# TheJacksonLaboratory/cnn_autoencoder

Measured on AMD Instinct MI355X. Metric: tiles/sec, compress+decompress round trip of 1024x1024x3 histology tiles, higher is better.
Workload: dtype f32 (f16x3 split MFMA: 3 f16 MFMAs per product, fp32 accumulate)

## Files before the change

cnn_autoencoder_amd/csrc/cae_api.hip:

```cpp
#include "cae_hip.h"
#include "cae_internal.hpp"
#include "cae_kernels.hpp"
#include "cae_kernels_f16.hpp"
#include "cae_launch.hpp"
#include "cae_pack.hpp"

#include <algorithm>
#include <cmath>
#include <cstdio>
#include <cstdlib>
#include <cstring>
#include <string>

namespace cae {

thread_local std::string g_last_error;
thread_local int64_t g_last_ticket = 0;
thread_local int g_force_fp32 = 0;

int fail(int code, const char *fmt, ...) {
    char buf[512];
    va_list ap;
    va_start(ap, fmt);
    vsnprintf(buf, sizeof buf, fmt, ap);
// ... 74 lines not shown
            if (l.set && l.f16_bad) return false;
    return true;
}

Model::~Model() {
    if (order_event) (void)hipEventDestroy((hipEvent_t)order_event);
    if (flags) (void)hipHostFree(flags);
}

struct ProfScope {
    Model *m;
    int track;
    hipStream_t st;
    std::vector<std::pair<void *, void *>> ev;
    hipEvent_t cur = nullptr;
    ProfScope(Model *m_, int track_, hipStream_t st_) : m(m_), track(track_), st(st_) {}
    void begin() {
        if (!m->profiling) return;
        hipEvent_t a;
        if (hipEventCreate(&a) != hipSuccess) return;
        (void)hipEventRecord(a, st);
        cur = a;
    }
    void end() {
        if (!m->profiling || !cur) return;
        hipEvent_t b;
        if (hipEventCreate(&b) != hipSuccess) return;
        (void)hipEventRecord(b, st);
        ev.emplace_back((void *)cur, (void *)b);
        cur = nullptr;
    }
    ~ProfScope() {
        if (m->profiling && !ev.empty()) m->prof[track].push_back(std::move(ev));
    }
};

static unsigned ew_grid(size_t total) {
    size_t b = (total + 255) / 256;
    return (unsigned)std::min<size_t>(std::max<size_t>(b, 1), 256 * 8 * 4);
}

static int layer_of(Model *m, int track, int index, Layer *&l) {
    if (track != CAE_ANALYSIS && track != CAE_SYNTHESIS) return fail(CAE_ERR_ARG, "bad track %d", track);
    if (index < 0 || index >= m->L) return fail(CAE_ERR_ARG, "layer index %d out of range", index);
    l = &(track == CAE_ANALYSIS ? m->enc : m->dec)[index];
    return CAE_OK;
}

static int upload_channels(DevBuf &d, const float *v, int c, int ct, float fill) {
    if (!v) {
        d.reset();
        return CAE_OK;
    }
    return d.upload(pad_channels(v, c, ct, fill));
}

static LayerArgs layer_args(const Model *m, const float *in, int in_planes, void *out, int n, int h, int w, int oh, int ow,
                            int ct, int cout, int outfmt, int act, int *flag) {
    LayerArgs a{};
    a.in = in;
    a.out = out;
    a.zero = m->zero.get<float>();
    a.medians = m->zero.get<float>();
    a.flag = flag;
    a.N = n;
    a.H = h;
    a.W = w;
    a.OH = oh;
    a.OW = ow;
    a.in_planes = in_planes;
    a.out_planes = ct * 4;
    a.cout = cout;
    a.outfmt = outfmt;
    a.act = act;
    return a;
}

}

using namespace cae;

template <int R>
static void launch_likelihood(Model *m, const float *y, int n, int hw, float *yhat, float *lik, double *part,
                              hipStream_t st) {
    hipLaunchKernelGGL(likelihood_kernel<R>, dim3(m->c_bn, n), dim3(256), 0, st, y, m->medians_dev.get<float>(),
                       m->density_dev.get<float>(), m->density_per_channel, m->density_k, m->density_bound,
                       m->likelihood_plain, m->c_bn, hw, yhat, lik, part);
}

static int set_stage(Model *m, int track, Layer &l, int stage, const float *w, const float *bias, const float *beta,
                     const float *gamma, int act, int add_residual, int post_act) {
    const int ctin = round_ct(l.cin);
    if (ctin < 0) return fail(CAE_ERR_UNSUPPORTED, "more than 192 channels not supported");
    if ((int)l.stages.size() <= stage) l.stages.resize(stage + 1);
    Layer::Stage &sg = l.stages[stage];
    const bool tr = track == CAE_SYNTHESIS;
    CAE_TRY(sg.wp.upload(pack_weights(w, tr, l.cin, l.cin, m->ks, ctin, tr)));
    CAE_TRY(upload_channels(sg.bias, bias, l.cin, ctin, 0.0f));
    sg.gdn = beta != nullptr;
    if (sg.gdn) {
        CAE_TRY(upload_channels(sg.beta, beta, l.cin, ctin, 1.0f));
        CAE_TRY(sg.gp.upload(pack_gamma(gamma, l.cin, ctin)));
    }
    sg.act = act;
    sg.add_res = add_residual != 0;
    sg.post_act = post_act;
    if (m->precision == 1) {
// ... 970 lines not shown
```

cnn_autoencoder_amd/csrc/cae_kernels.hpp:

```cpp
#pragma once
#include <hip/hip_runtime.h>
#include <stdint.h>
#include <type_traits>
#include <utility>

namespace cae {

typedef float f32x16 __attribute__((ext_vector_type(16)));
typedef float f32x4 __attribute__((ext_vector_type(4)));

enum OutFmt { OUT_C8 = 0, OUT_NCHW = 1, OUT_U8HWC = 2, OUT_SYM = 3, OUT_PMAP = 4 };

struct LayerArgs {
    const float *in;
    void *out;
    const float *wp;
    const float *bias;
    const float *gp;
    const float *beta;
    const float *zero;
    int N, H, W, OH, OW;
    int in_planes;
    int cci;
    int out_planes;
    int cout;
    int tiles_x, tiles_y;
    int outfmt;
    int act;
    const float *res;
    int res_planes;
    int post_act;
    const float *medians;
    const void *pm;
    int *flag;
};

__device__ __forceinline__ uint8_t clip_u8(float q) {
    return (uint8_t)__builtin_fmaxf(__builtin_fminf(q, 255.0f), 0.0f);
}
__device__ __forceinline__ int round_sym(float d) {
    return (int)rintf(__builtin_fminf(__builtin_fmaxf(d, -1073741824.0f), 1073741824.0f));
}

template <int N, class F, int... I>
__device__ __forceinline__ void static_for_impl(F &&f, std::integer_sequence<int, I...>) {
    (f(std::integral_constant<int, I>{}), ...);
}
template <int N, class F>
__device__ __forceinline__ void static_for(F &&f) {
    static_for_impl<N>(static_cast<F &&>(f), std::make_integer_sequence<int, N>{});
}

__device__ __forceinline__ int reflect_idx(int i, int n) {
    i = i < 0 ? -i : i;
    i = i >= n ? 2 * n - 2 - i : i;
    i = i < 0 ? 0 : i;
    return i >= n ? n - 1 : i;
}

__device__ __forceinline__ void glds16(const void *gsrc, void *lds_wave_base) {
    __builtin_amdgcn_global_load_lds((const __attribute__((address_space(1))) void *)gsrc,
                                     (__attribute__((address_space(3))) void *)lds_wave_base, 16, 0, 0);
}

__device__ __forceinline__ void wait_vm0() { asm volatile("s_waitcnt vmcnt(0)" ::: "memory"); }

__device__ __forceinline__ constexpr int acc_row(int r) { return (r & 3) + 8 * (r >> 2); }

template <int CT>
__device__ __forceinline__ void init_acc(f32x16 (&acc)[CT], const float *vec, int h, float fill) {
#pragma unroll
    for (int ct = 0; ct < CT; ++ct)
#pragma unroll
        for (int r = 0; r < 16; ++r) acc[ct][r] = vec ? vec[32 * ct + acc_row(r) + 4 * h] : fill;
}

template <int CT, int NW, bool INVERSE, int STAGE_BYTES, class Tail>
__device__ __forceinline__ void gdn_stages(f32x16 (&y)[CT], const LayerArgs &p, char *smem, int &sc,
                                           int wave, int lane, Tail tail) {
    constexpr int G_BYTES = CT * 4096;
    const int h = lane >> 5;
    f32x16 nrm[CT];
    init_acc<CT>(nrm, p.beta, h, 1.0f);
#pragma unroll
    for (int jt = 0; jt < CT; ++jt) {
        wait_vm0();
        __syncthreads();
        char *cur = smem + (sc & 1) * STAGE_BYTES;
        char *nxt = smem + ((sc + 1) & 1) * STAGE_BYTES;
        const char *gb = cur + lane * 16;
        f32x4 g_cur[CT];
#pragma unroll
        for (int co = 0; co < CT; ++co) g_cur[co] = *(const f32x4 *)(gb + (co * 4) * 1024);
        if (jt + 1 < CT) {
            const char *src = (const char *)p.gp + (size_t)(jt + 1) * G_BYTES;
#pragma unroll
            for (int i = 0; i < (CT * 4 + NW - 1) / NW; ++i) {
                const int j = wave + i * NW;
                if (j < CT * 4) glds16(src + j * 1024 + lane * 16, nxt + j * 1024);
            }
        } else {
            tail(nxt);
        }
#pragma unroll
        for (int q = 0; q < 4; ++q) {
            f32x4 g_nxt[CT];
            if (q + 1 < 4) {
#pragma unroll
                for (int co = 0; co < CT; ++co) g_nxt[co] = *(const f32x4 *)(gb + (co * 4 + q + 1) * 1024);
            }
            __builtin_amdgcn_sched_barrier(0);
#pragma unroll
            for (int jj = 0; jj < 4; ++jj) {
                const float v = y[jt][4 * q + jj];
                const float sq = v * v;
#pragma unroll
                for (int co = 0; co < CT; ++co)
                    nrm[co] = __builtin_amdgcn_mfma_f32_32x32x2f32(g_cur[co][jj], sq, nrm[co], 0, 0, 0);
            }
            if (q + 1 < 4) {
#pragma unroll
                for (int co = 0; co < CT; ++co) g_cur[co] = g_nxt[co];
            }
        }
        ++sc;
    }
#pragma unroll
// ... 1087 lines not shown
```

cnn_autoencoder_amd/csrc/cae_kernels_f16.hpp:

```cpp
#pragma once
#include "cae_kernels.hpp"

namespace cae {

constexpr int F16_ISSUERS = 2;
#define ISSUER(w, NW, NI) ((w) < (NI) ? (w) : -1)

typedef _Float16 f16x8 __attribute__((ext_vector_type(8)));
typedef _Float16 f16x4 __attribute__((ext_vector_type(4)));


__device__ __forceinline__ void split_f16(float v, _Float16 &hi, _Float16 &lo) {
    hi = (_Float16)v;
    lo = (_Float16)(v - (float)hi);
}

typedef unsigned u32x2v __attribute__((ext_vector_type(2)));
__device__ __forceinline__ u32x2v split2_f16(float a, float b) {
    typedef float f32x2 __attribute__((ext_vector_type(2)));
    typedef _Float16 f16x2 __attribute__((ext_vector_type(2)));
    const f32x2 ab = {a, b};
    const unsigned hi = __builtin_bit_cast(unsigned, __builtin_convertvector(ab, f16x2));
    float l0, l1;
    asm("v_fma_mix_f32 %0, %1, -1.0, %2 op_sel_hi:[1,0,0]" : "=v"(l0) : "v"(hi), "v"(a));
// ... 292 lines not shown
    int sc = 0;

    issue_stage(0, std::integral_constant<int, 0>{}, smem);
    for (int q = 0; q < p.cci; ++q) {
        static_for<KS>([&](auto ky_tag) {
            constexpr int ky = decltype(ky_tag)::value;
            wait_vm0();
            __syncthreads();
            char *cur = smem + (sc & 1) * STAGE_BYTES;
            char *nxt = smem + ((sc + 1) & 1) * STAGE_BYTES;
            if constexpr (ky + 1 < KS) {
                issue_stage(q, std::integral_constant<int, ky + 1>{}, nxt);
            } else {
                if (q + 1 < p.cci) {
                    issue_stage(q + 1, std::integral_constant<int, 0>{}, nxt);
                } else if (GDN) {
                    issue_gamma0<CT, NW>(p, nxt, wave, lane);
                }
            }
            const char *wb = cur + lane * 16;
            const char *hb = cur + b_off;
#pragma unroll
            for (int kx = 0; kx < KS; ++kx) {
                const int kxr = kx;
                f16x8 bh[PT], bl[PT];
#pragma unroll
                for (int pt = 0; pt < PT; ++pt) {
                    bh[pt] = *(const f16x8 *)(hb + pt * B_PT + kxr * 16);
                    bl[pt] = *(const f16x8 *)(hb + pt * B_PT + kxr * 16 + B_HL);
                }
#pragma unroll
                for (int ct = 0; ct < CT; ++ct) {
                    const f16x8 ah = *(const f16x8 *)(wb + ((kxr * CT + ct) * 2 + 0) * 1024);
                    const f16x8 al = *(const f16x8 *)(wb + ((kxr * CT + ct) * 2 + 1) * 1024);
#pragma unroll
                    for (int pt = 0; pt < PT; ++pt) acc[pt][ct] = mfma3(ah, al, bh[pt], bl[pt], acc[pt][ct]);
                }
            }
            ++sc;
        });
    }

    if constexpr (GDN) {
        gdn_stages_f16<CT, PT, NW, ZP, STAGE_BYTES>(acc, p, smem, sc, wave, lane, [](char *) {});
    }
#pragma unroll
    for (int pt = 0; pt < PT; ++pt) {
        const int oy = oy0 + 2 * PT * wave + 2 * pt + (m >> 4), ox = ox0 + (m & 15);
        store_tiles_f16<CT, SP, (GDN ? 0 : 1) | (RES ? 2 : 0)>(acc[pt], p, n, oy, ox, h, oy < p.OH && ox < p.OW);
    }
}

template <int CT, bool INVERSE>
__device__ __forceinline__ void gdn_resident_f16(f32x16 (&y)[CT], const char *gbuf, const float *beta_lds, int lane) {
    const int h = lane >> 5;
    f32x16 nrm[CT];
    float mx = 0.0f;
#pragma unroll
    for (int ct = 0; ct < CT; ++ct)
#pragma unroll
        for (int r = 0; r < 16; r += 2)
            mx = absmax3(mx, y[ct][r], y[ct][r + 1]);
    float isc;
    const float sc = pixel_scale(mx, &isc), sc2 = sc * sc;
#pragma unroll
    for (int ct = 0; ct < CT; ++ct)
#pragma unroll
        for (int r = 0; r < 16; ++r) nrm[ct][r] = beta_lds[32 * ct + acc_row(r) + 4 * h] * sc2;
#pragma unroll
    for (int jt = 0; jt < CT; ++jt) {
        const char *gb = gbuf + jt * (CT * 4096) + lane * 16;
#pragma unroll
        for (int s = 0; s < 2; ++s) {
            __builtin_amdgcn_sched_barrier(0);
            u32x4v hw, lw;
#pragma unroll
            for (int e = 0; e < 4; ++e) {
                const float v0 = y[jt][8 * s + 2 * e] * sc, v1 = y[jt][8 * s + 2 * e + 1] * sc;
                { const u32x2v t_ = split2_f16(v0 * v0, v1 * v1); hw[e] = t_[0]; lw[e] = t_[1]; }
                if constexpr (!INVERSE) {
                    y[jt][8 * s + 2 * e] = v0;
                    y[jt][8 * s + 2 * e + 1] = v1;
                }
            }
            const f16x8 sh = __builtin_bit_cast(f16x8, hw), sl = __builtin_bit_cast(f16x8, lw);
#pragma unroll
            for (int co = 0; co < CT; ++co) {
                if (co & 1) __builtin_amdgcn_sched_barrier(0);
                const f16x8 gh = *(const f16x8 *)(gb + ((co * 2 + s) * 2 + 0) * 1024);
                const f16x8 gl = *(const f16x8 *)(gb + ((co * 2 + s) * 2 + 1) * 1024);
                nrm[co] = mfma3(gh, gl, sh, sl, nrm[co]);
            }
        }
    }
#pragma unroll
    for (int ct = 0; ct < CT; ++ct)
#pragma unroll
        for (int r = 0; r < 16; ++r) {
            const float nv = nrm[ct][r];
            if constexpr (INVERSE)
                y[ct][r] *= __builtin_amdgcn_sqrtf(nv) * isc;
            else
                y[ct][r] *= __builtin_amdgcn_rsqf(nv);
        }
}

template <int CT, bool INVERSE>
__device__ __forceinline__ void gdn_resident_pipe_f16(f32x16 (&y)[CT], const char *gbuf, const float *beta_lds, int lane) {
    const int h = lane >> 5;
    f32x16 nrm[CT];
    float mx = 0.0f;
#pragma unroll
    for (int ct = 0; ct < CT; ++ct)
#pragma unroll
        for (int r = 0; r < 16; r += 2)
            mx = absmax3(mx, y[ct][r], y[ct][r + 1]);
    float isc;
    const float sc = pixel_scale(mx, &isc), sc2 = sc * sc;
#pragma unroll
    for (int ct = 0; ct < CT; ++ct)
#pragma unroll
// ... 55 lines not shown
                y[ct][r] *= __builtin_amdgcn_rsqf(nv);
        }
}

template <int CT, bool INVERSE, bool SP>
__global__ void __launch_bounds__(256, 1) gdn_f16_kernel(const LayerArgs p) {
    constexpr int NW = 4;
    extern __shared__ __attribute__((aligned(16))) char smem[];
    char *gbuf = smem;
    float *beta_lds = (float *)(smem + CT * CT * 4096);
    const int lane = threadIdx.x & 63;
    const int wave = __builtin_amdgcn_readfirstlane(threadIdx.x >> 6);
    const int h = lane >> 5, m = lane & 31;
    for (int j = wave; j < CT * CT * 4; j += NW) glds16((const char *)p.gp + (size_t)j * 1024 + lane * 16, gbuf + j * 1024);
    for (int i = threadIdx.x; i < CT * 32; i += NW * 64) beta_lds[i] = p.beta[i];
    wait_vm0();
    __syncthreads();

    const int groups = (int)(c8s_row_bytes<SP>(p.OW) / 1024);
    const long total = (long)p.N * p.OH * groups;
    const size_t row_bytes = c8s_row_bytes<SP>(p.OW);
    char *base = (char *)p.out;
    for (long t = (long)blockIdx.x * NW + wave; t < total; t += (long)gridDim.x * NW) {
        const int g = (int)(t % groups);
        const long rest = t / groups;
        const int oy = (int)(rest % p.OH), n = (int)(rest / p.OH);
        const int ox = SP ? (g >> 1) * 64 + 2 * m + (g & 1) : g * 32 + m;
        const bool valid = ox < p.OW;
        f32x16 y[CT];
#pragma unroll
        for (int ct = 0; ct < CT; ++ct)
#pragma unroll
            for (int pl = 0; pl < 4; ++pl) {
                const size_t row = ((size_t)n * p.out_planes + 4 * ct + pl) * p.OH + oy;
                const char *src = base + row * row_bytes + (size_t)g * 1024 + m * 16 + 8 * h;
                const f16x4 vh = *(const f16x4 *)src, vl = *(const f16x4 *)(src + 512);
#pragma unroll
                for (int k = 0; k < 4; ++k) y[ct][4 * pl + k] = valid ? (float)vh[k] + (float)vl[k] : 0.0f;
            }
        float mx = 0.0f;
#pragma unroll
        for (int ct = 0; ct < CT; ++ct)
#pragma unroll
            for (int r = 0; r < 16; r += 2)
                mx = absmax3(mx, y[ct][r], y[ct][r + 1]);
        float isc;
        const float sc = pixel_scale(mx, &isc), sc2 = sc * sc;
        constexpr int CH = CT / 2;
        static_assert(CT % 2 == 0, "channel tiles are halved");
#pragma unroll
        for (int half = 0; half < 2; ++half) {
            f32x16 nrm[CH];
#pragma unroll
            for (int c = 0; c < CH; ++c)
#pragma unroll
                for (int r = 0; r < 16; ++r) nrm[c][r] = beta_lds[32 * (half * CH + c) + acc_row(r) + 4 * h] * sc2;
#pragma unroll
            for (int jt = 0; jt < CT; ++jt) {
                const char *gb = gbuf + jt * (CT * 4096) + lane * 16;
#pragma unroll
                for (int s2 = 0; s2 < 2; ++s2) {
                    __builtin_amdgcn_sched_barrier(0);
                    u32x4v hw, lw;
#pragma unroll
                    for (int e = 0; e < 4; ++e) {
                        const float v0 = y[jt][8 * s2 + 2 * e] * sc, v1 = y[jt][8 * s2 + 2 * e + 1] * sc;
                        { const u32x2v t_ = split2_f16(v0 * v0, v1 * v1); hw[e] = t_[0]; lw[e] = t_[1]; }
                    }
                    const f16x8 sh = __builtin_bit_cast(f16x8, hw), sl = __builtin_bit_cast(f16x8, lw);
#pragma unroll
                    for (int c = 0; c < CH; ++c) {
                        const int co = half * CH + c;
                        const f16x8 gh = *(const f16x8 *)(gb + ((co * 2 + s2) * 2 + 0) * 1024);
                        const f16x8 gl = *(const f16x8 *)(gb + ((co * 2 + s2) * 2 + 1) * 1024);
                        nrm[c] = mfma3(gh, gl, sh, sl, nrm[c]);
                    }
                }
            }
#pragma unroll
            for (int c = 0; c < CH; ++c)
#pragma unroll
                for (int r = 0; r < 16; ++r) {
                    const float nv = nrm[c][r];
                    nrm[c][r] = y[half * CH + c][r] * (INVERSE ? __builtin_amdgcn_sqrtf(nv) : __builtin_amdgcn_rsqf(nv)) *
                                (INVERSE ? isc : sc);
                }
            if (valid) store_split_f16<CH, SP>(nrm, p, n, oy, ox, h, half * CH);
        }
    }
}

template <int KS, int CT, bool GDN>
struct FirstGeomF16 {
    static constexpr int NW = 8;
    static constexpr int PAD = KS / 2;
    static constexpr int TX = 16, TY = 2 * NW;
    static constexpr int WH = 2 * TX + KS - 2, HH = 2 * TY + KS - 2;
    static constexpr int NS = (KS * KS + 3) / 4;
    static constexpr int W_BYTES = NS * CT * 2048;
    static constexpr int G_BYTES = GDN ? CT * CT * 4096 : 0;
    static constexpr int RH = KS + 2;
    static constexpr int WAVE_HALO_BYTES = ((RH * WH * 16 + 1023) / 1024) * 1024;
    static constexpr int VEC_BYTES = 1024 + ((2 * CT * 32 * 4 + 1023) / 1024) * 1024;
    static constexpr int FIXED_BYTES = G_BYTES + W_BYTES + VEC_BYTES;
    static constexpr int LDS_BYTES = FIXED_BYTES + NW * WAVE_HALO_BYTES;
    static constexpr int NPOS = (RH * WH + 63) / 64;
};

template <int KS, int CT, bool GDN, bool U8>
// ... 78 lines not shown

    const char *hb = whalo + ((2 * (m >> 4)) * WH + 2 * (m & 15)) * 16;
    const char *wb = wbuf + lane * 16;
    for (; t < total; t += gridDim.x) {
        const int tn = t + gridDim.x;
        const bool has_next = tn < total;
        if (has_next) fetch(tn);

        const int n = t / tiles_img, rem = t - n * tiles_img;
        const int ty = rem / p.tiles_x, tx = rem - ty * p.tiles_x;
        f32x16 acc[CT];
#pragma unroll
        for (int ct = 0; ct < CT; ++ct)
#pragma unroll
            for (int r = 0; r < 16; ++r) acc[ct][r] = bias_lds[32 * ct + acc_row(r) + 4 * h];
#pragma unroll
        for (int s = 0; s < NS; ++s) {
            u32x4v bhw, blw;
#pragma unroll
            for (int half = 0; half < 2; ++half) {
                const int t0 = 4 * s + half, t1 = 4 * s + 2 + half;
                const int o0 = t0 < KS * KS ? ((t0 / KS) * WH + (t0 % KS)) * 16 : -1;
                const int o1 = t1 < KS * KS ? ((t1 / KS) * WH + (t1 % KS)) * 16 : -1;
                f32x4 v0 = {0.f, 0.f, 0.f, 0.f}, v1 = {0.f, 0.f, 0.f, 0.f};
                if (o0 >= 0) v0 = *(const f32x4 *)(hb + o0);
                if (o1 >= 0) v1 = *(const f32x4 *)(hb + o1);
                const f32x4 v = h ? v1 : v0;
                { const u32x2v t_ = split2_f16(v[0], v[1]); bhw[2 * half] = t_[0]; blw[2 * half] = t_[1]; }
                { const u32x2v t_ = split2_f16(v[2], v[3]); bhw[2 * half + 1] = t_[0]; blw[2 * half + 1] = t_[1]; }
            }
            const f16x8 bh = __builtin_bit_cast(f16x8, bhw), bl = __builtin_bit_cast(f16x8, blw);
#pragma unroll
            for (int ct = 0; ct < CT; ++ct) {
                const f16x8 ah = *(const f16x8 *)(wb + ((s * CT + ct) * 2 + 0) * 1024);
                const f16x8 al = *(const f16x8 *)(wb + ((s * CT + ct) * 2 + 1) * 1024);
                acc[ct] = mfma3(ah, al, bh, bl, acc[ct]);
            }
        }
        __builtin_amdgcn_wave_barrier();
        if (has_next) commit();
        __builtin_amdgcn_wave_barrier();
        if constexpr (GDN) gdn_resident_pipe_f16<CT, false>(acc, gbuf, beta_lds, lane);
        const int oy = ty * TY + 2 * wave + (m >> 4), ox = tx * TX + (m & 15);
        store_tiles_f16<CT, false, !GDN>(acc, p, n, oy, ox, h, oy < p.OH && ox < p.OW);
    }
    if constexpr (!U8)
        if (bad) *p.flag = 1;
}

__host__ __device__ __forceinline__ size_t pmap_record(int n, int OH, int OW, int oy, int ox) {
    return ((((size_t)n * OH + oy) * 2 + (ox & 1)) * (OW >> 1) + (ox >> 1)) * 32;
}

template <int CT>
__device__ __forceinline__ void store_pmap_f16(const f32x16 (&y)[CT], const LayerArgs &p, char *tbuf, int n, int oy, int par,
                                               int j0, int lane, bool row_valid) {
    const int h = lane >> 5, m = lane & 31;
    f32x16 pm;
#pragma unroll
    for (int r = 0; r < 16; ++r) pm[r] = 0.0f;
    float mx = 0.0f;
    const char *ab = (const char *)p.pm + lane * 16;
#pragma unroll
    for (int jt = 0; jt < CT; ++jt)
#pragma unroll
        for (int s = 0; s < 2; ++s) {
            u32x4v hw, lw;
#pragma unroll
            for (int e = 0; e < 4; ++e) {
                const float v0 = y[jt][8 * s + 2 * e], v1 = y[jt][8 * s + 2 * e + 1];
                mx = absmax3(mx, v0, v1);
                const u32x2v t_ = split2_f16(v0, v1);
                hw[e] = t_[0];
                lw[e] = t_[1];
            }
            const f16x8 sh = __builtin_bit_cast(f16x8, hw), sl = __builtin_bit_cast(f16x8, lw);
            const f16x8 ah = *(const f16x8 *)(ab + ((jt * 2 + s) * 2 + 0) * 1024);
            const f16x8 al = *(const f16x8 *)(ab + ((jt * 2 + s) * 2 + 1) * 1024);
            pm = mfma3(ah, al, sh, sl, pm);
        }
    raise_if_over(mx, p.flag);
    __builtin_amdgcn_wave_barrier();
#pragma unroll
    for (int g = 0; g < 4; ++g) {
        const f32x4 v = {pm[4 * g], pm[4 * g + 1], pm[4 * g + 2], pm[4 * g + 3]};
        *(f32x4 *)(tbuf + m * 128 + (((2 * g + h) ^ (m & 7)) * 16)) = v;
    }
    __builtin_amdgcn_wave_barrier();
    const int half_w = p.OW >> 1;
    float *row = (float *)p.out + ((((size_t)n * p.OH + oy) * 2 + par) * half_w) * 32;
#pragma unroll
    for (int it = 0; it < 4; ++it) {
        const int px = (lane >> 3) + 8 * it, q = lane & 7;
        const f32x4 v = *(const f32x4 *)(tbuf + px * 128 + ((q ^ (px & 7)) * 16));
        if (row_valid && j0 + px < half_w) *(f32x4 *)(row + (size_t)(j0 + px) * 32 + 4 * q) = v;
    }
    __builtin_amdgcn_wave_barrier();
}

static __global__ void __launch_bounds__(256) pmap_gather_kernel(const float *pm, const float *bias, void *out, int N, int H,
                                                               int W, int cout, int fmt, int tiles_x, int tiles_y) {
    constexpr int T = 16, R = T + 1, PITCH = 36;
    __shared__ __attribute__((aligned(16))) float rec[R * R * PITCH];
    __shared__ __attribute__((aligned(4))) uint8_t orow[2 * T][2 * T * 3 + 4];
    int bid = blockIdx.x;
    const int tx = bid % tiles_x;
    bid /= tiles_x;
    const int ty = bid % tiles_y;
    const int n = bid / tiles_y;
    const int a0 = ty * T, b0 = tx * T;
    constexpr int NIT = (R * R * 8 + 255) / 256;
    f32x4 stage[NIT];
#pragma unroll
    for (int it = 0; it < NIT; ++it) {
        const int i = threadIdx.x + it * 256;
        const int q = i & 7, r = i >> 3;
        const int ra = r / R, rb = r - ra * R;
        const int a = a0 + ra, b = b0 + rb;
        stage[it] = f32x4{0.0f, 0.0f, 0.0f, 0.0f};
        if (i < R * R * 8 && a < H && b < W) stage[it] = *(const f32x4 *)(pm + pmap_record(n, H, W, a, b) + 4 * q);
    }
#pragma unroll
    for (int it = 0; it < NIT; ++it) {
        const int i = threadIdx.x + it * 256;
        if (i < R * R * 8) *(f32x4 *)(rec + (i >> 3) * PITCH + 4 * (i & 7)) = stage[it];
    }
    __syncthreads();
    const int la = threadIdx.x >> 4, lb = threadIdx.x & 15;
    const int a = a0 + la, b = b0 + lb;
    const float *p00 = rec + (la * R + lb) * PITCH, *p01 = p00 + PITCH, *p10 = p00 + R * PITCH, *p11 = p10 + PITCH;
    const int OH = 2 * H, OW = 2 * W;
    const bool u8 = fmt == OUT_U8HWC;
    typedef float f32x2 __attribute__((ext_vector_type(2)));
    const f32x4 s0 = *(const f32x4 *)(p00), s1 = *(const f32x4 *)(p00 + 4), s2 = *(const f32x4 *)(p00 + 8);
    const f32x4 l0 = *(const f32x4 *)(p01 + 12), u0 = *(const f32x4 *)(p10 + 20), d0 = *(const f32x4 *)(p11 + 28);
    const f32x2 l1 = *(const f32x2 *)(p01 + 16), u1 = *(const f32x2 *)(p10 + 24);
    const float self[12] = {s0[0], s0[1], s0[2], s0[3], s1[0], s1[1], s1[2], s1[3], s2[0], s2[1], s2[2], s2[3]};
    const float left[6] = {l0[0], l0[1], l0[2], l0[3], l1[0], l1[1]};
    const float up[6] = {u0[0], u0[1], u0[2], u0[3], u1[0], u1[1]};
    const float diag[3] = {d0[0], d0[1], d0[2]};
#pragma unroll
    for (int c = 0; c < 3; ++c) {
        if (c >= cout) break;
        const float bs = bias ? bias[c] : 0.0f;
        const float o00 = bs + self[c];
        const float o01 = bs + self[3 + c] + left[c];
        const float o10 = bs + self[6 + c] + up[c];
        const float o11 = bs + self[9 + c] + left[3 + c] + up[3 + c] + diag[c];
// ... 4 lines not shown
            orow[2 * la + 1][(2 * lb + 1) * cout + c] = clip_u8(o11 * 255.0f);
        } else if (a < H && b < W) {
            float *o = (float *)out + (((size_t)n * cout + c) * OH + 2 * a) * OW + 2 * b;
            o[0] = o00;
            o[1] = o01;
            o[OW] = o10;
            o[OW + 1] = o11;
        }
    }
    if (!u8) return;
    __syncthreads();
    const int row_bytes = 2 * T * cout;
    const int valid_rows = min(2 * T, OH - 2 * a0), valid_bytes = min(2 * T, OW - 2 * b0) * cout;
    uint8_t *obase = (uint8_t *)out + (((size_t)n * OH + 2 * a0) * OW + 2 * b0) * cout;
    const bool dwords = ((((size_t)OW * cout) & 3) == 0) && (((uintptr_t)obase & 3) == 0) && (row_bytes & 3) == 0 &&
                        valid_bytes == row_bytes;
    if (dwords) {
        const int per_row = row_bytes / 4;
        for (int i = threadIdx.x; i < valid_rows * per_row; i += 256) {
            const int r = i / per_row, q = i - r * per_row;
            *(uint32_t *)(obase + (size_t)r * OW * cout + 4 * q) = *(const uint32_t *)(&orow[r][4 * q]);
        }
    } else {
        for (int i = threadIdx.x; i < valid_rows * valid_bytes; i += 256) {
            const int r = i / valid_bytes, q = i - r * valid_bytes;
            obase[(size_t)r * OW * cout + q] = orow[r][q];
        }
    }
}

template <int KS, int CT, int NW, int PT, bool IGDN>
struct DeconvGeomF16 {
    static constexpr int P = KS / 2;
    static constexpr int DLO = -((P + 1) / 2), DHI = (KS - 1 - P) / 2;
    static constexpr int WH = 32 + DHI - DLO;
    static constexpr int ROWS = NW * PT;
    static constexpr int NSTRAY = WH - 32;
    static constexpr int AL_INSTR = 4 * ROWS * 32 / 64;
    static constexpr int AL_BYTES = AL_INSTR * 1024;
    static constexpr int STRAY_INSTR = (NSTRAY * 4 * ROWS + 63) / 64;
    static constexpr int HALO_INSTR = AL_INSTR + STRAY_INSTR;
    static_assert((4 * ROWS * 32) % 64 == 0 && 64 % (4 * ROWS) == 0, "halo image assumes 4, 8 or 16 input rows per block");
    static constexpr int W_INSTR = KS * CT * 2;
    static constexpr int W_BYTES = W_INSTR * 1024;
    static constexpr int G_BYTES = IGDN ? CT * 4096 : 0;
    static constexpr int CONV_STAGE = W_BYTES + HALO_INSTR * 1024;
    static constexpr int STAGE_BYTES = CONV_STAGE > G_BYTES ? CONV_STAGE : G_BYTES;
    static constexpr int NI = NW / F16_ISSUERS > 0 ? NW / F16_ISSUERS : 1;
    static constexpr int MAXP = (HALO_INSTR + NI - 1) / NI;
    static constexpr int AL_PER = AL_INSTR / NI, AL_STEP = NI * 64 / (ROWS * 32);
    static_assert(AL_INSTR % NI == 0 && (NI * 64) % (ROWS * 32) == 0 && AL_STEP <= 2 && STRAY_INSTR <= NI,
                  "issuer waves must each cover whole (plane, half) images of the aligned halo");
    static constexpr int G_ALL = IGDN ? CT * CT * 4096 : 0;
    static constexpr bool RESIDENT = IGDN && 2 * STAGE_BYTES + G_ALL <= 160 * 1024;
    static constexpr int PMAP_LDS = NW * 4096;
    static constexpr bool TBUF_IN_STAGE = RESIDENT && 2 * STAGE_BYTES + G_ALL + PMAP_LDS > 160 * 1024;
    static_assert(!TBUF_IN_STAGE || STAGE_BYTES >= PMAP_LDS, "transpose buffers must fit a stage buffer");
    static constexpr int lds_bytes(bool pmap) {
        return 2 * STAGE_BYTES + (RESIDENT ? G_ALL : 0) + ((pmap && !TBUF_IN_STAGE) ? PMAP_LDS : 0);
    }
    static constexpr int dmin(int py) { return -((py + P) / 2); }
    static constexpr int nky(int py) { return (KS - 1 - py - P) / 2 - dmin(py) + 1; }
};

template <int KS, int CT, int NW, int PT, bool IGDN, int PY>
__device__ __forceinline__ void deconv_issue_f16(const LayerArgs &p, const char *in_n, size_t plane_bytes, int s,
                                                 char *buf, const int *hrow, const int *hbase, int wave, int lane) {
    using G = DeconvGeomF16<KS, CT, NW, PT, IGDN>;
    constexpr int NKY = G::nky(PY);
    const int q = s / NKY, d = G::dmin(PY) + (s - q * NKY);
    const int ky = 2 * d + PY + G::P;
    if (ISSUER(wave, NW, G::NI) < 0) return;
    const int iw = ISSUER(wave, NW, G::NI);
    const char *wsrc = (const char *)p.wp + (size_t)(q * KS + ky) * G::W_BYTES;
#pragma unroll
    for (int i = 0; i < (G::W_INSTR + G::NI - 1) / G::NI; ++i) {
        const int j = iw + i * G::NI;
        if (j < G::W_INSTR) glds16(wsrc + j * 1024 + lane * 16, buf + j * 1024);
    }
    const char *planes = in_n + (size_t)(2 * q) * plane_bytes;
    const size_t row_bytes = c8s_row_bytes<true>(p.W);
    {
        const int iy = hrow[0] - d;
        const bool ok = iy >= 0 && iy < p.H && hbase[0] >= 0;
        const char *src = planes + hbase[0] + (size_t)iy * row_bytes;
#pragma unroll
        for (int i = 0; i < G::AL_PER; ++i) {
            constexpr int K = G::AL_STEP;
            const char *g = ok ? src + (size_t)((i * K) >> 1) * plane_bytes + ((i * K) & 1) * 512 : (const char *)p.zero;
            glds16(g, buf + G::W_BYTES + (iw + i * G::NI) * 1024);
        }
    }
    if (iw < G::STRAY_INSTR) {
        const int iy = hrow[1] - d;
        const bool ok = iy >= 0 && iy < p.H && hbase[1] >= 0;
        const char *g = ok ? planes + hbase[1] + (size_t)iy * row_bytes : (const char *)p.zero;
        glds16(g, buf + G::W_BYTES + (G::AL_INSTR + iw) * 1024);
    }
}

template <int KS, int CT, int NW, int PT, bool IGDN, int PY>
__device__ __forceinline__ void deconv_phase_f16(const LayerArgs &p, const char *in_n, size_t plane_bytes, char *smem,
                                                 int &sc, const int *hrow, const int *hbase, int wave, int lane,
                                                 const int (&b_off)[KS], int stray_mask, int n, int iy, int ix) {
    using G = DeconvGeomF16<KS, CT, NW, PT, IGDN>;
    constexpr int P = G::P;
    constexpr int STAGE_BYTES = G::STAGE_BYTES;
    const int h = lane >> 5;
    const int NS = p.cci * G::nky(PY);
    f32x16 acc[2][PT][CT];
#pragma unroll
    for (int x = 0; x < 2; ++x)
#pragma unroll
        for (int pt = 0; pt < PT; ++pt) init_acc<CT>(acc[x][pt], p.bias, h, 0.0f);

    for (int s = 0; s < NS; ++s) {
        wait_vm0();
        __syncthreads();
        char *cur = smem + (sc & 1) * STAGE_BYTES;
        char *nxt = smem + ((sc + 1) & 1) * STAGE_BYTES;
        if (s + 1 < NS) {
            deconv_issue_f16<KS, CT, NW, PT, IGDN, PY>(p, in_n, plane_bytes, s + 1, nxt, hrow, hbase, wave, lane);
        } else if (IGDN && !G::RESIDENT) {
            issue_gamma0<CT, NW>(p, nxt, wave, lane);
        } else if (PY == 0) {
            deconv_issue_f16<KS, CT, NW, PT, IGDN, 1>(p, in_n, plane_bytes, 0, nxt, hrow, hbase, wave, lane);
        }
        const char *wb = cur + lane * 16;
#pragma unroll
        for (int kx = 0; kx < KS; ++kx) {
            if (PT > 1) __builtin_amdgcn_sched_barrier(0);
            const int px = (kx + P) & 1;
            f16x8 bh[PT], bl[PT];
            const bool stray = (stray_mask >> kx) & 1;
            const int b_hl = stray ? G::ROWS * 16 : G::ROWS * 32 * 16, b_pt = stray ? 16 : 32 * 16;
#pragma unroll
            for (int pt = 0; pt < PT; ++pt) {
                bh[pt] = *(const f16x8 *)(cur + b_off[kx] + pt * b_pt);
                bl[pt] = *(const f16x8 *)(cur + b_off[kx] + pt * b_pt + b_hl);
            }
#pragma unroll
            for (int ct = 0; ct < CT; ++ct) {
                const int ctr = ct;
                const f16x8 ah = *(const f16x8 *)(wb + ((kx * CT + ctr) * 2 + 0) * 1024);
                const f16x8 al = *(const f16x8 *)(wb + ((kx * CT + ctr) * 2 + 1) * 1024);
#pragma unroll
                for (int pt = 0; pt < PT; ++pt) {
                    if (px == 0)
                        acc[0][pt][ct] = mfma3(ah, al, bh[pt], bl[pt], acc[0][pt][ct]);
                    else
                        acc[1][pt][ct] = mfma3(ah, al, bh[pt], bl[pt], acc[1][pt][ct]);
                }
            }
        }
        ++sc;
    }

    char *tbuf = smem + 2 * STAGE_BYTES + (G::RESIDENT ? G::G_ALL : 0) + wave * 4096;
    if constexpr (G::TBUF_IN_STAGE) {
        __syncthreads();
        tbuf = smem + ((sc + 1) & 1) * STAGE_BYTES + wave * 4096;
    }
    auto store = [&](auto x_tag, auto pt_tag) {
        constexpr int x = decltype(x_tag)::value, pt = decltype(pt_tag)::value;
        if (p.outfmt == OUT_PMAP)
            store_pmap_f16<CT>(acc[x][pt], p, tbuf, n, 2 * (iy + pt) + PY, x, ix - (lane & 31), lane, (iy + pt) < p.H);
        else
            store_tiles_f16<CT, true, !IGDN && CT <= 4>(acc[x][pt], p, n, 2 * (iy + pt) + PY, 2 * ix + x, h, (iy + pt) < p.H && ix < p.W);
    };
    if constexpr (IGDN && G::RESIDENT) {
        const char *gbuf = smem + 2 * STAGE_BYTES;
        static_for<2 * PT>([&](auto it) {
            constexpr int idx = decltype(it)::value;
            constexpr int x = idx / PT, pt = idx % PT;
            gdn_resident_f16<CT, true>(acc[x][pt], gbuf, p.beta, lane);
            store(std::integral_constant<int, x>{}, std::integral_constant<int, pt>{});
        });
    } else if constexpr (IGDN) {
        static_for<2 * PT>([&](auto it) {
            constexpr int idx = decltype(it)::value;
            constexpr int x = idx / PT, pt = idx % PT;
            gdn_stages_f16<CT, PT, NW, true, STAGE_BYTES, pt, 1>(acc[x], p, smem, sc, wave, lane, [&](char *nxt) {
                if constexpr (idx + 1 < 2 * PT) {
                    issue_gamma0<CT, NW>(p, nxt, wave, lane);
                } else if (PY == 0) {
                    deconv_issue_f16<KS, CT, NW, PT, IGDN, 1>(p, in_n, plane_bytes, 0, nxt, hrow, hbase, wave, lane);
                }
            });
            store(std::integral_constant<int, x>{}, std::integral_constant<int, pt>{});
        });
    } else {
        static_for<2 * PT>([&](auto it) {
            constexpr int idx = decltype(it)::value;
            store(std::integral_constant<int, idx / PT>{}, std::integral_constant<int, idx % PT>{});
        });
    }
}

template <int KS, int CT, int NW, int PT, bool IGDN>
__global__ void __launch_bounds__(NW * 64, NW * PT <= 4 ? 2 : 1) deconv_s2_f16_kernel(const LayerArgs p) {
    using G = DeconvGeomF16<KS, CT, NW, PT, IGDN>;
    extern __shared__ __attribute__((aligned(16))) char smem[];
    const int lane = threadIdx.x & 63;
    const int wave = __builtin_amdgcn_readfirstlane(threadIdx.x >> 6);
    const int h = lane >> 5, m = lane & 31;
    int bid = xcd_tile_order(blockIdx.x, gridDim.x);
    const int tx = bid % p.tiles_x;
    bid /= p.tiles_x;
    const int ty = bid % p.tiles_y;
    const int n = bid / p.tiles_y;
    const int iy0 = ty * G::ROWS, ix0 = tx * 32;

    int hrow[2], hbase[2];
    {
        const int iw = ISSUER(wave, NW, G::NI) < 0 ? 0 : ISSUER(wave, NW, G::NI);
        const int plane_i = (int)((size_t)p.H * c8s_row_bytes<true>(p.W));
        const int pc = iw * 64 + lane;
        int plhl = pc / (G::ROWS * 32);
        int ixp = ix0 + (pc & 31);
        hrow[0] = iy0 + (pc / 32) % G::ROWS;
        hbase[0] = ixp < p.W ? (plhl >> 1) * plane_i + (int)c8s_piece<true>(ixp) + (plhl & 1) * 512 : -1;
        int js = iw * (64 / (4 * G::ROWS)) + lane / (4 * G::ROWS);
        js = js < G::NSTRAY ? js : G::NSTRAY - 1;
        plhl = (lane / G::ROWS) & 3;
        ixp = ix0 + (js < G::DHI ? js : 32 + js) - G::DHI;
        hrow[1] = iy0 + lane % G::ROWS;
        hbase[1] = (ixp >= 0 && ixp < p.W) ? (plhl >> 1) * plane_i + (int)c8s_piece<true>(ixp) + (plhl & 1) * 512 : -1;
    }
    const size_t plane_bytes = (size_t)p.H * c8s_row_bytes<true>(p.W);
    const char *in_n = (const char *)p.in + (size_t)n * p.in_planes * plane_bytes;
    int b_off[KS], stray_mask = 0;
#pragma unroll
    for (int kx = 0; kx < KS; ++kx) {
        const int pxk = (kx + G::P) & 1, dx = (kx - G::P - pxk) / 2;
        const int c = m + G::DHI - dx, row = PT * wave;
        if (c >= G::DHI && c < G::DHI + 32) {
            b_off[kx] = G::W_BYTES + (((2 * h) * G::ROWS + row) * 32 + c - G::DHI) * 16;
        } else {
            const int js = c < G::DHI ? c : c - 32;
            b_off[kx] = G::W_BYTES + G::AL_BYTES + ((js * 4 + 2 * h) * G::ROWS + row) * 16;
            stray_mask |= 1 << kx;
        }
    }
    const int iy = iy0 + PT * wave, ix = ix0 + m;
    int sc = 0;
    if constexpr (G::RESIDENT) {
        for (int j = wave; j < G::G_ALL / 1024; j += NW)
            glds16((const char *)p.gp + (size_t)j * 1024 + lane * 16, smem + 2 * G::STAGE_BYTES + j * 1024);
    }
    deconv_issue_f16<KS, CT, NW, PT, IGDN, 0>(p, in_n, plane_bytes, 0, smem, hrow, hbase, wave, lane);
    deconv_phase_f16<KS, CT, NW, PT, IGDN, 0>(p, in_n, plane_bytes, smem, sc, hrow, hbase, wave, lane, b_off, stray_mask, n,
                                              iy, ix);
    deconv_phase_f16<KS, CT, NW, PT, IGDN, 1>(p, in_n, plane_bytes, smem, sc, hrow, hbase, wave, lane, b_off, stray_mask, n,
                                              iy, ix);
}

template <int KS, int NW_, int DEPTH_>
struct LastGeomF16 {
    static constexpr int NW = NW_, DEPTH = DEPTH_;
    static constexpr int P = KS / 2;
    static constexpr int DLO = -((P + 1) / 2), DHI = (KS - 1 - P) / 2;
    static constexpr int NB = DHI - DLO + 1;
    static constexpr int TXC = 32, NT = TXC / 16;
    static constexpr int WH = TXC + NB - 1, HR = NW + NB - 1;
    static constexpr int PLANE_PIECES = HR * WH;
    static constexpr int HALO_PIECES = 8 * PLANE_PIECES;
    static constexpr int MAXP = ((HALO_PIECES + 63) / 64 + NW - 1) / NW;
    static constexpr int STAGE_BYTES = MAXP * NW * 1024;
    static constexpr int lds_bytes(int nq) { return DEPTH * STAGE_BYTES + NB * NB * nq * 2048; }
};

template <int KS, int NW, int DEPTH>
__global__ void __launch_bounds__(NW * 64, 1) deconv_last_f16_kernel(const LayerArgs p) {
    using G = LastGeomF16<KS, NW, DEPTH>;
    constexpr int DLO = G::DLO, DHI = G::DHI, NB = G::NB, NT = G::NT, WH = G::WH, HR = G::HR;
    constexpr int PLANE_PIECES = G::PLANE_PIECES, MAXP = G::MAXP, STAGE_BYTES = G::STAGE_BYTES;
    extern __shared__ __attribute__((aligned(16))) char smem[];
    const int lane = threadIdx.x & 63;
    const int wave = __builtin_amdgcn_readfirstlane(threadIdx.x >> 6);
    const int g = lane >> 4, col = lane & 15;
    const int nq = p.cci;
    char *wbuf = smem + DEPTH * STAGE_BYTES;

    const int tiles_img = p.tiles_x * p.tiles_y;
    const int total = p.N * tiles_img;
    const size_t row_bytes = c8s_row_bytes<true>(p.W);
    const size_t plane_bytes = (size_t)p.H * row_bytes;

    int pc_r[MAXP], pc_x[MAXP], pc_ghl[MAXP];
#pragma unroll
    for (int i = 0; i < MAXP; ++i) {
        int pc = (wave + i * NW) * 64 + lane;
        pc = pc < G::HALO_PIECES ? pc : G::HALO_PIECES - 1;
        pc_ghl[i] = pc / PLANE_PIECES;
        const int rem = pc - pc_ghl[i] * PLANE_PIECES;
        pc_r[i] = rem / WH;
        pc_x[i] = rem - pc_r[i] * WH;
    }
    auto issue = [&](int step) {
        const int it = step / nq, q = step - it * nq;
        const long t = (long)blockIdx.x + (long)it * gridDim.x;
        char *buf = smem + (step % DEPTH) * STAGE_BYTES;
        const bool live = t < total;
// ... 162 lines not shown
```

Baseline: 4089.

## Stage bias/beta and pmap weights in LDS, vectorize per-channel vector loads

Per-channel bias and beta vectors are now read with 16-byte vector loads instead of scalar gathers, and the host checks that the device buffers are aligned for this. In the f16 deconvolution kernel, bias and beta are copied into LDS when they fit, and as many probability-map weight tiles as the leftover LDS allows are prefetched with global_load_lds. The pmap store also computes its row base once with readfirstlane. The aim is to cut repeated global reads of small constant vectors and weights in the epilogue, at the cost of more LDS per block, which may lower occupancy, plus an extra block-wide sync.

New measurement: 4167 (median of 6 runs). +1.9%, better.

```diff
diff --git a/cnn_autoencoder_amd/csrc/cae_api.hip b/cnn_autoencoder_amd/csrc/cae_api.hip
--- a/cnn_autoencoder_amd/csrc/cae_api.hip
+++ b/cnn_autoencoder_amd/csrc/cae_api.hip
@@ -150,7 +150,11 @@
         d.reset();
         return CAE_OK;
     }
-    return d.upload(pad_channels(v, c, ct, fill));
+    CAE_TRY(d.upload(pad_channels(v, c, ct, fill)));
+    if ((uintptr_t)d.p % 16 != 0 || d.bytes != (size_t)ct * 32 * sizeof(float))
+        return fail(CAE_ERR_HIP, "per-channel vector: device buffer %p (%zu bytes) is not a 16-byte aligned run of %d floats",
+                    d.p, d.bytes, ct * 32);
+    return CAE_OK;
 }
 
 static LayerArgs layer_args(const Model *m, const float *in, int in_planes, void *out, int n, int h, int w, int oh, int ow,
diff --git a/cnn_autoencoder_amd/csrc/cae_kernels.hpp b/cnn_autoencoder_amd/csrc/cae_kernels.hpp
--- a/cnn_autoencoder_amd/csrc/cae_kernels.hpp
+++ b/cnn_autoencoder_amd/csrc/cae_kernels.hpp
@@ -67,12 +67,26 @@
 
 __device__ __forceinline__ constexpr int acc_row(int r) { return (r & 3) + 8 * (r >> 2); }
 
+__device__ __forceinline__ void load_acc_tile(f32x16 &a, const float *vec, int ct, int h) {
+#pragma unroll
+    for (int g = 0; g < 4; ++g) {
+        const f32x4 v = *(const f32x4 *)(vec + 32 * ct + 8 * g + 4 * h);
+#pragma unroll
+        for (int k = 0; k < 4; ++k) a[4 * g + k] = v[k];
+    }
+}
+
 template <int CT>
 __device__ __forceinline__ void init_acc(f32x16 (&acc)[CT], const float *vec, int h, float fill) {
 #pragma unroll
-    for (int ct = 0; ct < CT; ++ct)
-#pragma unroll
-        for (int r = 0; r < 16; ++r) acc[ct][r] = vec ? vec[32 * ct + acc_row(r) + 4 * h] : fill;
+    for (int ct = 0; ct < CT; ++ct) {
+        if (vec) {
+            load_acc_tile(acc[ct], vec, ct, h);
+        } else {
+#pragma unroll
+            for (int r = 0; r < 16; ++r) acc[ct][r] = fill;
+        }
+    }
 }
 
 template <int CT, int NW, bool INVERSE, int STAGE_BYTES, class Tail>
diff --git a/cnn_autoencoder_amd/csrc/cae_kernels_f16.hpp b/cnn_autoencoder_amd/csrc/cae_kernels_f16.hpp
--- a/cnn_autoencoder_amd/csrc/cae_kernels_f16.hpp
+++ b/cnn_autoencoder_amd/csrc/cae_kernels_f16.hpp
@@ -368,7 +368,7 @@
 }
 
 template <int CT, bool INVERSE>
-__device__ __forceinline__ void gdn_resident_f16(f32x16 (&y)[CT], const char *gbuf, const float *beta_lds, int lane) {
+__device__ __forceinline__ void gdn_resident_f16(f32x16 (&y)[CT], const char *gbuf, const float *beta, int lane) {
     const int h = lane >> 5;
     f32x16 nrm[CT];
     float mx = 0.0f;
@@ -380,9 +380,11 @@
     float isc;
     const float sc = pixel_scale(mx, &isc), sc2 = sc * sc;
 #pragma unroll
-    for (int ct = 0; ct < CT; ++ct)
-#pragma unroll
-        for (int r = 0; r < 16; ++r) nrm[ct][r] = beta_lds[32 * ct + acc_row(r) + 4 * h] * sc2;
+    for (int ct = 0; ct < CT; ++ct) {
+        load_acc_tile(nrm[ct], beta, ct, h);
+#pragma unroll
+        for (int r = 0; r < 16; ++r) nrm[ct][r] *= sc2;
+    }
 #pragma unroll
     for (int jt = 0; jt < CT; ++jt) {
         const char *gb = gbuf + jt * (CT * 4096) + lane * 16;
@@ -544,9 +546,11 @@
         for (int half = 0; half < 2; ++half) {
             f32x16 nrm[CH];
 #pragma unroll
-            for (int c = 0; c < CH; ++c)
-#pragma unroll
-                for (int r = 0; r < 16; ++r) nrm[c][r] = beta_lds[32 * (half * CH + c) + acc_row(r) + 4 * h] * sc2;
+            for (int c = 0; c < CH; ++c) {
+                load_acc_tile(nrm[c], beta_lds, half * CH + c, h);
+#pragma unroll
+                for (int r = 0; r < 16; ++r) nrm[c][r] *= sc2;
+            }
 #pragma unroll
             for (int jt = 0; jt < CT; ++jt) {
                 const char *gb = gbuf + jt * (CT * 4096) + lane * 16;
@@ -731,19 +735,19 @@
     return ((((size_t)n * OH + oy) * 2 + (ox & 1)) * (OW >> 1) + (ox >> 1)) * 32;
 }
 
-template <int CT>
+template <int CT, int LDS_JT>
 __device__ __forceinline__ void store_pmap_f16(const f32x16 (&y)[CT], const LayerArgs &p, char *tbuf, int n, int oy, int par,
-                                               int j0, int lane, bool row_valid) {
+                                               int j0, int lane, bool row_valid, const char *pm_lds) {
     const int h = lane >> 5, m = lane & 31;
     f32x16 pm;
 #pragma unroll
     for (int r = 0; r < 16; ++r) pm[r] = 0.0f;
     float mx = 0.0f;
-    const char *ab = (const char *)p.pm + lane * 16;
 #pragma unroll
     for (int jt = 0; jt < CT; ++jt)
 #pragma unroll
         for (int s = 0; s < 2; ++s) {
+            const char *ab = (jt < LDS_JT ? pm_lds : (const char *)p.pm) + lane * 16;
             u32x4v hw, lw;
 #pragma unroll
             for (int e = 0; e < 4; ++e) {
@@ -766,13 +770,13 @@
         *(f32x4 *)(tbuf + m * 128 + (((2 * g + h) ^ (m & 7)) * 16)) = v;
     }
     __builtin_amdgcn_wave_barrier();
-    const int half_w = p.OW >> 1;
-    float *row = (float *)p.out + ((((size_t)n * p.OH + oy) * 2 + par) * half_w) * 32;
+    const int half_w = p.OW >> 1, j0u = __builtin_amdgcn_readfirstlane(j0);
+    float *rec0 = (float *)p.out + ((((size_t)n * p.OH + oy) * 2 + par) * half_w + j0u) * 32 + 4 * lane;
 #pragma unroll
     for (int it = 0; it < 4; ++it) {
         const int px = (lane >> 3) + 8 * it, q = lane & 7;
         const f32x4 v = *(const f32x4 *)(tbuf + px * 128 + ((q ^ (px & 7)) * 16));
-        if (row_valid && j0 + px < half_w) *(f32x4 *)(row + (size_t)(j0 + px) * 32 + 4 * q) = v;
+        if (row_valid && j0u + px < half_w) *(f32x4 *)(rec0 + it * 256) = v;
     }
     __builtin_amdgcn_wave_barrier();
 }
@@ -883,12 +887,20 @@
     static_assert(AL_INSTR % NI == 0 && (NI * 64) % (ROWS * 32) == 0 && AL_STEP <= 2 && STRAY_INSTR <= NI,
                   "issuer waves must each cover whole (plane, half) images of the aligned halo");
     static constexpr int G_ALL = IGDN ? CT * CT * 4096 : 0;
+    static constexpr int VEC_BYTES = 2 * CT * 128;
     static constexpr bool RESIDENT = IGDN && 2 * STAGE_BYTES + G_ALL <= 160 * 1024;
+    static constexpr int G_LDS = RESIDENT ? G_ALL : 0;
     static constexpr int PMAP_LDS = NW * 4096;
-    static constexpr bool TBUF_IN_STAGE = RESIDENT && 2 * STAGE_BYTES + G_ALL + PMAP_LDS > 160 * 1024;
+    static constexpr bool TBUF_IN_STAGE = RESIDENT && 2 * STAGE_BYTES + G_LDS + PMAP_LDS > 160 * 1024;
     static_assert(!TBUF_IN_STAGE || STAGE_BYTES >= PMAP_LDS, "transpose buffers must fit a stage buffer");
+    static constexpr bool VEC_IN_LDS = 2 * STAGE_BYTES + G_LDS + VEC_BYTES + (TBUF_IN_STAGE ? 0 : PMAP_LDS) <= 160 * 1024;
+    static constexpr int VEC_LDS = VEC_IN_LDS ? VEC_BYTES : 0;
+    static constexpr int TBUF_LDS = TBUF_IN_STAGE ? 0 : PMAP_LDS;
+    static constexpr int PM_ROOM = (160 * 1024 - (2 * STAGE_BYTES + G_LDS + VEC_LDS + TBUF_LDS)) / 4096;
+    static constexpr int PM_LDS_JT = PM_ROOM < 0 ? 0 : (PM_ROOM < CT ? PM_ROOM : CT);
+    static constexpr int PM_OFF = 2 * STAGE_BYTES + G_LDS + VEC_LDS + TBUF_LDS;
     static constexpr int lds_bytes(bool pmap) {
-        return 2 * STAGE_BYTES + (RESIDENT ? G_ALL : 0) + ((pmap && !TBUF_IN_STAGE) ? PMAP_LDS : 0);
+        return 2 * STAGE_BYTES + G_LDS + VEC_LDS + (pmap ? TBUF_LDS + PM_LDS_JT * 4096 : 0);
     }
     static constexpr int dmin(int py) { return -((py + P) / 2); }
     static constexpr int nky(int py) { return (KS - 1 - py - P) / 2 - dmin(py) + 1; }
@@ -939,11 +951,14 @@
     constexpr int STAGE_BYTES = G::STAGE_BYTES;
     const int h = lane >> 5;
     const int NS = p.cci * G::nky(PY);
+    const float *vec_lds = (const float *)(smem + 2 * STAGE_BYTES + G::G_LDS);
+    const float *bias = G::VEC_IN_LDS ? vec_lds : p.bias;
+    [[maybe_unused]] const float *beta = G::VEC_IN_LDS ? vec_lds + CT * 32 : p.beta;
     f32x16 acc[2][PT][CT];
 #pragma unroll
     for (int x = 0; x < 2; ++x)
 #pragma unroll
-        for (int pt = 0; pt < PT; ++pt) init_acc<CT>(acc[x][pt], p.bias, h, 0.0f);
+        for (int pt = 0; pt < PT; ++pt) init_acc<CT>(acc[x][pt], bias, h, 0.0f);
 
     for (int s = 0; s < NS; ++s) {
         wait_vm0();
@@ -987,7 +1002,7 @@
         ++sc;
     }
 
-    char *tbuf = smem + 2 * STAGE_BYTES + (G::RESIDENT ? G::G_ALL : 0) + wave * 4096;
+    char *tbuf = smem + 2 * STAGE_BYTES + G::G_LDS + G::VEC_LDS + wave * 4096;
     if constexpr (G::TBUF_IN_STAGE) {
         __syncthreads();
         tbuf = smem + ((sc + 1) & 1) * STAGE_BYTES + wave * 4096;
@@ -995,7 +1010,8 @@
     auto store = [&](auto x_tag, auto pt_tag) {
         constexpr int x = decltype(x_tag)::value, pt = decltype(pt_tag)::value;
         if (p.outfmt == OUT_PMAP)
-            store_pmap_f16<CT>(acc[x][pt], p, tbuf, n, 2 * (iy + pt) + PY, x, ix - (lane & 31), lane, (iy + pt) < p.H);
+            store_pmap_f16<CT, G::PM_LDS_JT>(acc[x][pt], p, tbuf, n, 2 * (iy + pt) + PY, x, ix - (lane & 31), lane,
+                                             (iy + pt) < p.H, smem + G::PM_OFF);
         else
             store_tiles_f16<CT, true, !IGDN && CT <= 4>(acc[x][pt], p, n, 2 * (iy + pt) + PY, 2 * ix + x, h, (iy + pt) < p.H && ix < p.W);
     };
@@ -1004,7 +1020,7 @@
         static_for<2 * PT>([&](auto it) {
             constexpr int idx = decltype(it)::value;
             constexpr int x = idx / PT, pt = idx % PT;
-            gdn_resident_f16<CT, true>(acc[x][pt], gbuf, p.beta, lane);
+            gdn_resident_f16<CT, true>(acc[x][pt], gbuf, beta, lane);
             store(std::integral_constant<int, x>{}, std::integral_constant<int, pt>{});
         });
     } else if constexpr (IGDN) {
@@ -1079,7 +1095,19 @@
         for (int j = wave; j < G::G_ALL / 1024; j += NW)
             glds16((const char *)p.gp + (size_t)j * 1024 + lane * 16, smem + 2 * G::STAGE_BYTES + j * 1024);
     }
+    if (G::PM_LDS_JT > 0 && p.outfmt == OUT_PMAP) {
+        for (int j = wave; j < G::PM_LDS_JT * 4; j += NW)
+            glds16((const char *)p.pm + (size_t)j * 1024 + lane * 16, smem + G::PM_OFF + j * 1024);
+    }
     deconv_issue_f16<KS, CT, NW, PT, IGDN, 0>(p, in_n, plane_bytes, 0, smem, hrow, hbase, wave, lane);
+    if constexpr (G::VEC_IN_LDS) {
+        float *vec_lds = (float *)(smem + 2 * G::STAGE_BYTES + G::G_LDS);
+        for (int i = threadIdx.x; i < CT * 32; i += NW * 64) {
+            vec_lds[i] = p.bias ? p.bias[i] : 0.0f;
+            vec_lds[CT * 32 + i] = (IGDN && p.beta) ? p.beta[i] : 1.0f;
+        }
+        __syncthreads();
+    }
     deconv_phase_f16<KS, CT, NW, PT, IGDN, 0>(p, in_n, plane_bytes, smem, sc, hrow, hbase, wave, lane, b_off, stray_mask, n,
                                               iy, ix);
     deconv_phase_f16<KS, CT, NW, PT, IGDN, 1>(p, in_n, plane_bytes, smem, sc, hrow, hbase, wave, lane, b_off, stray_mask, n,
```
